# AndrewJarrett/raytracing-with-zig

Measured on NVIDIA B200. Metric: Msamples/s, higher is better.
Workload: dtype f32

## Files before the change

raytracing-with-zig_b200/csrc/rtz_api.cu:

```cuda
#include <cuda_runtime.h>
#include <dlfcn.h>
#include <nccl.h>

#include <algorithm>
#include <cerrno>
#include <cmath>
#include <cstdint>
#include <cstdio>
#include <cstdlib>
#include <cstring>
#include <condition_variable>
#include <functional>
#include <map>
#include <mutex>
#include <thread>
#include <memory>
#include <string>
#include <vector>

#include "../../include/rtz.h"
#include "rtz_kernels.cuh"
#include "rtz_bvh.cuh"
#include "rtz_scene.cuh"

// ... 193 lines not shown
    RTZ_CUDA(ctx->accum.reserve(3 * n_local_pixels));
    rtz::TraceParams P;
    P.cam = to_dev_camera(*cam, seed);
    P.sh = sg;
    P.geom = ctx->geom.p, P.pairs = ctx->pairs.p, P.aux = ctx->aux.p, P.albedo = ctx->albedo.p, P.wexp = ctx->wexp.p;
    P.orig = nullptr;
    P.n_spheres = ctx->n_spheres, P.n_pad = ctx->n_pad;
    pick_chunks(ctx, P, n_local_pixels);
    P.accum = ctx->accum.p;
    P.counter = ctx->counters.p;
    P.stats = ctx->counters.p + 1;
    {
        P.wave_shade_min = P.wave_regen_min = ctx->n_pad <= 32 ? 16u : ctx->n_pad <= 64 ? 12u : 8u;
        auto rcp = [](uint64_t d) -> unsigned long long {
            return d <= 1 ? 0ull : (unsigned long long)(((unsigned __int128)1 << 64) / d) + 1ull;
        };
        P.rcp_tile_pixels = rcp(sg.tile_pixels), P.rcp_tiles_x = rcp(sg.tiles_x), P.rcp_tile_w = rcp(sg.tile_w);
        P.rcp_chunks_per_pixel = rcp(P.chunks_per_pixel);
        if (const char* e = std::getenv("RTZ_WAVE_SHADE_MIN")) P.wave_shade_min = (uint32_t)std::min(32, std::max(1, std::atoi(e)));
        if (const char* e = std::getenv("RTZ_WAVE_REGEN_MIN")) P.wave_regen_min = (uint32_t)std::min(32, std::max(1, std::atoi(e)));
    }
    P.timeline = nullptr;
    if (const char* e = std::getenv("RTZ_TIMELINE")) {
        if (e[0] == '1') {
            RTZ_CUDA(ctx->timeline.reserve(4 * 65536));
            RTZ_CUDA(cudaMemsetAsync(ctx->timeline.p, 0, 4 * 65536 * sizeof(unsigned long long), ctx->stream));
            P.timeline = ctx->timeline.p;
        }
    }
    P.pool = nullptr, P.pool_count = reinterpret_cast<unsigned int*>(ctx->counters.p + 8);
    const char* de = std::getenv("RTZ_DRAIN");
    const bool drain = cam->mode == RTZ_MODE_PATH && ctx->variant != 4 && P.cam.bounce_max > 0 && !(de && de[0] == '0');
    if (drain) {
        RTZ_CUDA(ctx->pool.reserve(4ull * 64 * 32 * (size_t)ctx->sm_count * 2));
        P.pool = ctx->pool.p;
    }
    const bool use_const = ctx->n_pad <= rtz::kMaxConstSpheres && ctx->geo_const;
    const size_t smem = use_const ? 0 : (size_t)ctx->n_pad * 32;
    cudaFuncAttributes fa{};
    RTZ_CUDA(cudaFuncGetAttributes(&fa, rtz::trace_kernel_smem<512, 1>));
    const bool use_global = !use_const && smem + fa.sharedSizeBytes + 1024 > ctx->smem_optin;
    RTZ_CUDA(cudaEventRecord(ctx->ev[0], ctx->stream));
    RTZ_CUDA(cudaMemsetAsync(ctx->accum.p, 0, 3 * n_local_pixels * sizeof(unsigned long long), ctx->stream));
    RTZ_CUDA(cudaMemsetAsync(ctx->counters.p, 0, 16 * sizeof(unsigned long long), ctx->stream));
    RTZ_CUDA(cudaEventRecord(ctx->ev[1], ctx->stream));
    ctx->frame_launches = P.cam.bounce_max == 0 ? 1 : 2;
    int32_t rc = RTZ_OK;
    if (P.cam.bounce_max == 0) {
    } else if (cam->mode == RTZ_MODE_PATH_BVH) {
        rtz::BvhParams B{P, ctx->bvh_nodes.p, ctx->bvh_order.p, ctx->wexp.p};
        rc = launch_trace(ctx, rtz::trace_kernel_bvh<128, 6>, B, P.n_chunks, 128, 0);
    } else if (use_const) {
        static thread_local rtz::TraceParamsConst C;
        C.p = P;
        std::memcpy(C.pairs, ctx->h_pairs.data(), (size_t)ctx->n_pad * sizeof(float4));
        const bool wave_ok = P.n_chunks <= 0xFFFFFFFFull;
        if (ctx->variant == 4)
            rc = launch_trace(ctx, rtz::trace_kernel_const_parked<4, 128, 6>, C, P.n_chunks, 128, 0);
        else if (ctx->variant == 1)
            rc = launch_trace(ctx, rtz::trace_kernel_const<256, 3>, C, P.n_chunks, 256, 0);
        else if (ctx->variant == 2)
            rc = launch_trace(ctx, rtz::trace_kernel_const<128, 5>, C, P.n_chunks, 128, 0);
        else if (ctx->variant == 6)
            rc = launch_trace(ctx, rtz::trace_kernel_const<128, 7>, C, P.n_chunks, 128, 0);
        else if (ctx->variant == 7)
            rc = launch_trace(ctx, rtz::trace_kernel_const<128, 8>, C, P.n_chunks, 128, 0);
        else if (ctx->variant == 9 && wave_ok)
            rc = launch_trace(ctx, rtz::trace_kernel_wave<128, 10>, C, P.n_chunks, 128, 0);
        else if (ctx->variant == 10 && wave_ok)
            rc = launch_trace(ctx, rtz::trace_kernel_wave<128, 9>, C, P.n_chunks, 128, 0);
        else if (wave_ok && (ctx->variant == 8 || (ctx->variant == 0 && ctx->n_pad <= 32)))
            rc = launch_trace(ctx, rtz::trace_kernel_wave<128, 8>, C, P.n_chunks, 128, 0);
        else if (wave_ok && (ctx->variant == 12 || (ctx->variant == 0 && ctx->n_pad <= rtz::kMaxWaveSpheres)))
            rc = launch_trace(ctx, rtz::trace_kernel_wave_n<4, 128, 6>, C, P.n_chunks, 128, 0);
        else if (ctx->n_pad <= 64)
            rc = launch_trace(ctx, rtz::trace_kernel_const<128, 8>, C, P.n_chunks, 128, 0);
        else if (ctx->cull) {
            P.geom = ctx->rg_geom.p, P.aux = ctx->rg_aux.p, P.albedo = ctx->rg_albedo.p, P.wexp = ctx->rg_wexp.p;
            P.orig = ctx->rg_orig.p, P.pairs = nullptr;
            C.p = P;
            std::memcpy(C.pairs, ctx->h_rg_pairs.data(), (size_t)ctx->n_pad * sizeof(float4));
            std::memcpy(C.boxes, ctx->h_boxes.data(), ctx->h_boxes.size() * sizeof(float4));
            C.cull_r2 = ctx->cull_r2;
            rc = launch_trace(ctx, rtz::trace_kernel_const_cull<128, 6>, C, P.n_chunks, 128, 0);
        } else
            rc = launch_trace(ctx, rtz::trace_kernel_const<128, 6>, C, P.n_chunks, 128, 0);
    } else if (use_global) {
        rc = launch_trace(ctx, rtz::trace_kernel_global<128, 5>, P, P.n_chunks, 128, 0);
    } else {
        int occ[3] = {0, 0, 0};
        RTZ_CUDA(cudaFuncSetAttribute(rtz::trace_kernel_smem<128, 5>, cudaFuncAttributeMaxDynamicSharedMemorySize, (int)smem));
        RTZ_CUDA(cudaFuncSetAttribute(rtz::trace_kernel_smem<256, 2>, cudaFuncAttributeMaxDynamicSharedMemorySize, (int)smem));
        RTZ_CUDA(cudaFuncSetAttribute(rtz::trace_kernel_smem<512, 1>, cudaFuncAttributeMaxDynamicSharedMemorySize, (int)smem));
        RTZ_CUDA(cudaOccupancyMaxActiveBlocksPerMultiprocessor(&occ[0], rtz::trace_kernel_smem<128, 5>, 128, smem));
        RTZ_CUDA(cudaOccupancyMaxActiveBlocksPerMultiprocessor(&occ[1], rtz::trace_kernel_smem<256, 2>, 256, smem));
        RTZ_CUDA(cudaOccupancyMaxActiveBlocksPerMultiprocessor(&occ[2], rtz::trace_kernel_smem<512, 1>, 512, smem));
        const int warps[3] = {occ[0] * 4, occ[1] * 8, occ[2] * 16};
        int shape = 0;
        for (int k = 1; k < 3; ++k)
            if (warps[k] > warps[shape]) shape = k;
        if (ctx->variant >= 1 && ctx->variant <= 3) shape = ctx->variant - 1;
        switch (shape) {
            case 1: rc = launch_trace(ctx, rtz::trace_kernel_smem<256, 2>, P, P.n_chunks, 256, smem); break;
            case 2: rc = launch_trace(ctx, rtz::trace_kernel_smem<512, 1>, P, P.n_chunks, 512, smem); break;
            default: rc = launch_trace(ctx, rtz::trace_kernel_smem<128, 5>, P, P.n_chunks, 128, smem); break;
        }
    }
    if (rc != RTZ_OK) return rc;
    if (drain) {
        const unsigned blocks = (unsigned)ctx->sm_count * 8;
        if (ctx->n_spheres >= 64)
            rtz::drain_kernel<true><<<blocks, 128, 0, ctx->stream>>>(P);
        else
            rtz::drain_kernel<false><<<blocks, 128, 0, ctx->stream>>>(P);
        RTZ_CUDA(cudaGetLastError());
        ctx->frame_launches += 1;
    }
    RTZ_CUDA(cudaEventRecord(ctx->ev[2], ctx->stream));
    const uint64_t n3 = 3 * n_local_pixels;
    if (out.image)
        rtz::resolve_scatter_kernel<<<(unsigned)((n3 + 255) / 256), 256, 0, ctx->stream>>>(
            ctx->accum.p, sg, (uint32_t)cam->width, (uint32_t)cam->height, cam->pixel_samples_scale, out.image);
    else
        rtz::resolve_kernel<<<(unsigned)((n3 + 255) / 256), 256, 0, ctx->stream>>>(
            ctx->accum.p, n_local_pixels, cam->pixel_samples_scale, out.d_rgb, out.d_linear);
    RTZ_CUDA(cudaGetLastError());
    RTZ_CUDA(cudaEventRecord(ctx->ev[3], ctx->stream));
    RTZ_CUDA(cudaMemcpyAsync(ctx->h_counters, ctx->counters.p, 8 * sizeof(unsigned long long), cudaMemcpyDeviceToHost,
                             ctx->stream));
    return RTZ_OK;
}

int32_t collect_path(rtz_context* ctx, const rtz_camera* cam, const rtz::ShardGeom& sg, rtz_stats* st, uint64_t seed) {
    RTZ_CUDA(cudaStreamSynchronize(ctx->stream));
    if (const char* path = std::getenv("RTZ_TIMELINE_OUT")) {
        if (ctx->timeline.p && std::getenv("RTZ_TIMELINE") && std::getenv("RTZ_TIMELINE")[0] == '1') {
            std::vector<unsigned long long> h(4 * 65536);
            RTZ_CUDA(cudaMemcpy(h.data(), ctx->timeline.p, h.size() * sizeof(unsigned long long), cudaMemcpyDeviceToHost));
            if (FILE* f = std::fopen(path, "wb")) {
                std::fwrite(h.data(), sizeof(unsigned long long), h.size(), f);
                std::fclose(f);
            }
        }
    }
    if (st) {
        std::memset(st, 0, sizeof(*st));
        st->samples = ctx->h_counters[1], st->segments = ctx->h_counters[2];
        if (cam->bounce_max == 0) {
            uint64_t px = 0;
            for (uint32_t t = sg.rank; t < (uint64_t)sg.tiles_x * sg.tiles_y; t += sg.world) {
                const uint32_t ty = t / sg.tiles_x, tx = t - ty * sg.tiles_x;
                const uint64_t w = std::min<uint64_t>(sg.tile_w, cam->width - (uint64_t)tx * sg.tile_w);
                const uint64_t h = std::min<uint64_t>(sg.tile_h, cam->height - (uint64_t)ty * sg.tile_h);
                px += w * h;
            }
            st->samples = px * cam->samples_per_pixel;
        }
        st->depth_capped = ctx->h_counters[3], st->absorbed = ctx->h_counters[4];
        st->sphere_tests = cam->mode == RTZ_MODE_PATH_BVH ? ctx->h_counters[5] : st->segments * (uint64_t)ctx->n_spheres;
        st->nan_samples = ctx->h_counters[6];
        st->kernel_launches = ctx->frame_launches;
        st->gpus = 1;
        float ms = 0;
        cudaEventElapsedTime(&ms, ctx->ev[1], ctx->ev[2]), st->trace_ms = ms;
        cudaEventElapsedTime(&ms, ctx->ev[2], ctx->ev[3]), st->resolve_ms = ms;
        cudaEventElapsedTime(&ms, ctx->ev[0], ctx->ev[3]), st->total_ms = ms;
// ... 1096 lines not shown
```

raytracing-with-zig_b200/csrc/rtz_kernels.cuh:

```cuda
#pragma once
#include "rtz_device.cuh"

namespace rtz {

struct ShardGeom {
    uint32_t rank, world, tile_w, tile_h, tiles_x, tiles_y, n_local_tiles, tile_pixels;
};

struct TraceParams {
    DevCamera cam;
    ShardGeom sh;
    const float4* pairs;
    const float4* geom;
    const float4* aux;
    const float4* albedo;
    const float* wexp;
    const int* orig;
    int n_spheres;
    int n_pad;
    uint32_t chunk;
    uint32_t chunks_per_pixel;
    uint32_t n_local_pixels;
    uint64_t n_chunks;
    unsigned long long* accum;
    unsigned long long* counter;
    unsigned long long* stats;
    float4* pool;
    unsigned int* pool_count;
    unsigned long long* timeline;
    uint32_t wave_shade_min, wave_regen_min;
    unsigned long long rcp_tile_pixels, rcp_tiles_x, rcp_tile_w, rcp_chunks_per_pixel;
};

constexpr int kMaxConstSpheres = 512;
struct TraceParamsConst {
    TraceParams p;
    float4 pairs[kMaxConstSpheres];
    float4 boxes[2 * (kMaxConstSpheres / 32)];
    float cull_r2;
};

__device__ __forceinline__ bool local_to_global(const ShardGeom& s, uint32_t W, uint32_t H, uint32_t lp, uint32_t& x,
                                                uint32_t& y) {
    const uint32_t lt = lp / s.tile_pixels, within = lp - lt * s.tile_pixels;
    const uint32_t gt = lt * s.world + s.rank;
    const uint32_t ty = gt / s.tiles_x, tx = gt - ty * s.tiles_x;
    const uint32_t wy = within / s.tile_w, wx = within - wy * s.tile_w;
    x = tx * s.tile_w + wx, y = ty * s.tile_h + wy;
    return x < W && y < H && ty < s.tiles_y;
}

__device__ __forceinline__ uint32_t div_by(uint32_t n, unsigned long long rcp) {
    return rcp ? (uint32_t)__umul64hi((unsigned long long)n, rcp) : n;
}
__device__ __forceinline__ bool local_to_global_rcp(const ShardGeom& s, unsigned long long rcp_tile_pixels,
                                                    unsigned long long rcp_tiles_x, unsigned long long rcp_tile_w, uint32_t W,
                                                    uint32_t H, uint32_t lp, uint32_t& x, uint32_t& y) {
    const uint32_t lt = div_by(lp, rcp_tile_pixels), within = lp - lt * s.tile_pixels;
    const uint32_t gt = lt * s.world + s.rank;
    const uint32_t ty = div_by(gt, rcp_tiles_x), tx = gt - ty * s.tiles_x;
    const uint32_t wy = div_by(within, rcp_tile_w), wx = within - wy * s.tile_w;
    x = tx * s.tile_w + wx, y = ty * s.tile_h + wy;
    return x < W && y < H && ty < s.tiles_y;
}

__device__ __forceinline__ uint32_t smem_u32(const void* p) { return (uint32_t)__cvta_generic_to_shared(p); }
__device__ __forceinline__ void mbar_init(uint64_t* bar, uint32_t count) {
    asm volatile("mbarrier.init.shared::cta.b64 [%0], %1;" ::"r"(smem_u32(bar)), "r"(count));
}
__device__ __forceinline__ void mbar_expect_tx(uint64_t* bar, uint32_t bytes) {
    asm volatile("mbarrier.arrive.expect_tx.shared::cta.b64 _, [%0], %1;" ::"r"(smem_u32(bar)), "r"(bytes) : "memory");
}
__device__ __forceinline__ void bulk_g2s(void* dst, const void* src, uint32_t bytes, uint64_t* bar) {
    asm volatile("cp.async.bulk.shared::cluster.global.mbarrier::complete_tx::bytes [%0], [%1], %2, [%3];" ::"r"(
                     smem_u32(dst)),
                 "l"(src), "r"(bytes), "r"(smem_u32(bar))
                 : "memory");
}
__device__ __forceinline__ void mbar_wait(uint64_t* bar, uint32_t phase) {
    asm volatile(
        "{\n"
        ".reg .pred p;\n"
        "WAIT_%=:\n"
        "mbarrier.try_wait.parity.shared::cta.b64 p, [%0], %1;\n"
        "@p bra DONE_%=;\n"
        "bra WAIT_%=;\n"
        "DONE_%=:\n"
        "}\n" ::"r"(smem_u32(bar)),
        "r"(phase)
        : "memory");
}

struct Slot {
    Path path;
    RngKey key;
    uint32_t lp;
    bool alive;
};


__device__ __forceinline__ void resolve_candidates(const float4* __restrict__ gather, unsigned cand, int base, int cnt,
                                                   const Path& p, float tmin_d, float& closest, int& best,
                                                   const int* __restrict__ orig = nullptr) {
    while (cand) {
        const int bit = 31 - __clz(cand);
        cand &= ~(1u << bit);
        const int i = base + (cnt - 1 - bit);
        const float4 g = gather[i];
        candidate_root(g, g.w, i, p, tmin_d, closest, best, orig);
    }
}

__device__ __forceinline__ void test_pair(const float4 p0, const float4 p1, const Path& p, const RayK& k,
                                          unsigned& mask) {
    const float2 cx = make_float2(p0.x, p0.y), cy = make_float2(p0.z, p0.w);
    const float2 cz = make_float2(p1.x, p1.y), cw = make_float2(p1.z, p1.w);
    float2 h = __ffma2_rn(make_float2(p.dx, p.dx), cx, make_float2(k.k1, k.k1));
    h = __ffma2_rn(make_float2(p.dy, p.dy), cy, h);
    h = __ffma2_rn(make_float2(p.dz, p.dz), cz, h);
    float2 w = __ffma2_rn(make_float2(k.tx, k.tx), cx, make_float2(k.nk2, k.nk2));
    w = __ffma2_rn(make_float2(k.ty, k.ty), cy, w);
    w = __ffma2_rn(make_float2(k.tz, k.tz), cz, w);
    w = __fadd2_rn(w, cw);
    const float2 disc = __ffma2_rn(h, h, w);
    mask = __funnelshift_l(__float_as_uint(disc.x), mask, 1);
    mask = __funnelshift_l(__float_as_uint(disc.y), mask, 1);
}

__device__ __forceinline__ bool box_reach(const float4 b0, const float4 b1, const Path& p, float ix, float iy, float iz,
                                          float closest) {
    const float2 tx = __fmul2_rn(__fadd2_rn(make_float2(b0.x, b0.y), make_float2(-p.ox, -p.ox)), make_float2(ix, ix));
    const float2 ty = __fmul2_rn(__fadd2_rn(make_float2(b0.z, b0.w), make_float2(-p.oy, -p.oy)), make_float2(iy, iy));
    const float2 tz = __fmul2_rn(__fadd2_rn(make_float2(b1.x, b1.y), make_float2(-p.oz, -p.oz)), make_float2(iz, iz));
    const float tn = fmaxf(fmaxf(fminf(tx.x, tx.y), fminf(ty.x, ty.y)), fmaxf(fminf(tz.x, tz.y), 0.0f));
    const float tf = fminf(fminf(fmaxf(tx.x, tx.y), fmaxf(ty.x, ty.y)), fminf(fmaxf(tz.x, tz.y), closest));
    return tn <= tf;
}

template <bool kConstBank, bool kSkipSelf = false, bool kCull = false>
__device__ __forceinline__ void sweep2(const float4* __restrict__ pairs, const float4* __restrict__ gather, int n_pad,
                                       float tmin, float tmax, const Path& a, const Path& b, float& ta, int& ia,
                                       float& tb, int& ib, const float4* __restrict__ boxes = nullptr,
                                       float cull_r2 = 0.0f, const int* __restrict__ orig = nullptr) {
    RayK ka = ray_constants(a), kb = ray_constants(b);
    if (kConstBank && !kCull) asm volatile("" : "+f"(ka.tx), "+f"(ka.ty), "+f"(ka.tz), "+f"(kb.tx), "+f"(kb.ty), "+f"(kb.tz));
    float ca = tmax * a.len, cb = tmax * b.len;
    int ba = -1, bb = -1;
    float iax = 0.f, iay = 0.f, iaz = 0.f, ibx = 0.f, iby = 0.f, ibz = 0.f;
    if (kCull) {
        iax = 1.0f / a.dx, iay = 1.0f / a.dy, iaz = 1.0f / a.dz;
        ibx = 1.0f / b.dx, iby = 1.0f / b.dy, ibz = 1.0f / b.dz;
        if (!(-ka.nk2 <= cull_r2)) iax = iay = iaz = __int_as_float(0x7fffffff);
        if (!(-kb.nk2 <= cull_r2)) ibx = iby = ibz = __int_as_float(0x7fffffff);
    }
    for (int base = 0; base < n_pad; base += 32) {
        if (kCull && base > 0) {
            const float4 b0 = boxes[base >> 4], b1 = boxes[(base >> 4) + 1];
            const bool need = box_reach(b0, b1, a, iax, iay, iaz, ca) | box_reach(b0, b1, b, ibx, iby, ibz, cb);
            if (!__any_sync(0xFFFFFFFFu, need)) continue;
        }
        const int cnt = min(32, n_pad - base);
        unsigned ma = 0xFFFFFFFFu, mb = 0xFFFFFFFFu;
        const float4* g = pairs + base;
#pragma unroll 1
        for (int k = 0; k < cnt; k += 8) {
#pragma unroll
            for (int u = 0; u < 8; u += 2) {
                const float4 p0 = g[k + u], p1 = g[k + u + 1];
                test_pair(p0, p1, a, ka, ma);
                test_pair(p0, p1, b, kb, mb);
            }
        }
        unsigned canda = ~ma, candb = ~mb;
        if (kSkipSelf) {
            const unsigned ra = (unsigned)(a.self & ~kSelfLeaves) - (unsigned)base, rb = (unsigned)(b.self & ~kSelfLeaves) - (unsigned)base;
            if ((a.self >> 30) == 1 && ra < (unsigned)cnt) canda &= ~(1u << (cnt - 1 - (int)ra));
            if ((b.self >> 30) == 1 && rb < (unsigned)cnt) candb &= ~(1u << (cnt - 1 - (int)rb));
        }
        if (canda | candb) {
            float la = a.len, lb = b.len;
            if (!kConstBank) asm volatile("" : "+f"(la), "+f"(lb));
            resolve_candidates(gather, canda, base, cnt, a, tmin * la, ca, ba, orig);
            resolve_candidates(gather, candb, base, cnt, b, tmin * lb, cb, bb, orig);
        }
    }
    ta = ca, ia = ba, tb = cb, ib = bb;
}

__device__ __forceinline__ void finish_or_continue(const TraceParams& P, const float4* gather, const float4* s_aux,
                                                   const float4* s_alb, Slot& s, float t, int best,
                                                   unsigned long long& n_seg, uint32_t& n_samp, uint32_t& n_cap,
                                                   uint32_t& n_abs) {
    ++n_seg;
    float sr, sg, sb;
    int term;
    if (shade(P.cam, s.key, gather, s_aux, s_alb, s.path, t, best, sr, sg, sb, term)) {
        const unsigned long long fr = to_fixed(sr), fg = to_fixed(sg), fb = to_fixed(sb);
        unsigned long long* px = P.accum + 3ull * s.lp;
        if (fr) atomicAdd(px + 0, fr);
        if (fg) atomicAdd(px + 1, fg);
        if (fb) atomicAdd(px + 2, fb);
        if (sr != sr || sg != sg || sb != sb) atomicAdd(P.stats + 5, 1ULL);
        ++n_samp;
        n_cap += (term == 2), n_abs += (term == 1);
        s.alive = false;
    }
}

__device__ __forceinline__ void finish_or_continue(const TraceParams& P, const float4* gather, const float4* s_aux,
                                                   const float4* s_alb, Slot& s, float t, int best) {
    float sr, sg, sb;
    int term;
    if (shade(P.cam, s.key, gather, s_aux, s_alb, s.path, t, best, sr, sg, sb, term)) {
        const unsigned long long fr = to_fixed(sr), fg = to_fixed(sg), fb = to_fixed(sb);
        unsigned long long* px = P.accum + 3ull * s.lp;
        if (fr) atomicAdd(px + 0, fr);
        if (fg) atomicAdd(px + 1, fg);
        if (fb) atomicAdd(px + 2, fb);
        if (sr != sr || sg != sg || sb != sb) atomicAdd(P.stats + 5, 1ULL);
        if (term == 2) atomicAdd(P.stats + 2, 1ULL);
        if (term == 1) atomicAdd(P.stats + 3, 1ULL);
        s.alive = false;
    }
}

__device__ __forceinline__ unsigned long long globaltimer_ns() {
    unsigned long long t;
    asm volatile("mov.u64 %0, %globaltimer;" : "=l"(t));
    return t;
}

template <bool kUniform = false>
__device__ __forceinline__ void coop_hit(const float4* __restrict__ geom, const float* __restrict__ wexp,
                                         const int* __restrict__ orig, int n, float tmin, float tmax, const Path& mine,
                                         int src, unsigned lane, float& t_out, int& best_out) {
    Path q = mine;
    if (!kUniform) {
        q.ox = __shfl_sync(0xFFFFFFFFu, mine.ox, src), q.oy = __shfl_sync(0xFFFFFFFFu, mine.oy, src);
        q.oz = __shfl_sync(0xFFFFFFFFu, mine.oz, src), q.dx = __shfl_sync(0xFFFFFFFFu, mine.dx, src);
        q.dy = __shfl_sync(0xFFFFFFFFu, mine.dy, src), q.dz = __shfl_sync(0xFFFFFFFFu, mine.dz, src);
        q.len = __shfl_sync(0xFFFFFFFFu, mine.len, src), q.self = __shfl_sync(0xFFFFFFFFu, mine.self, src);
    }
    const float tmin_d = tmin * q.len;
    float closest = tmax * q.len;
    int best = -1;
    const RayK k = ray_constants(q);
    for (int base = (int)lane; base < n; base += 256) {
        unsigned cand = 0u;
#pragma unroll
        for (int j = 0; j < 8; ++j) {
            const int i = base + 32 * j;
            if (i < n) {
                const float4 g = __ldg(geom + i);
                const float d = expanded_disc(g.x, g.y, g.z, __ldg(wexp + i), q, k);
                cand |= (__float_as_uint(d) >> 31 ^ 1u) << j;
            }
        }
        while (cand) {
            const int j = __ffs(cand) - 1;
            cand &= cand - 1u;
            const int i = base + 32 * j;
            const float4 g = __ldg(geom + i);
            candidate_root(g, g.w, i, q, tmin_d, closest, best, orig);
        }
    }
#pragma unroll
    for (int o = 16; o > 0; o >>= 1) {
        const float t2 = __shfl_xor_sync(0xFFFFFFFFu, closest, o);
        const int b2 = __shfl_xor_sync(0xFFFFFFFFu, best, o);
        const bool tie_won = t2 == closest && b2 >= 0 && (best < 0 || (orig ? __ldg(orig + b2) < __ldg(orig + best) : b2 < best));
        if (t2 < closest || tie_won) closest = t2, best = b2;
    }
    if (kUniform || (int)lane == src) t_out = closest, best_out = best;
}

__device__ __forceinline__ void park_path(float4* __restrict__ e, const Slot& s) {
    const Path& p = s.path;
    e[0] = make_float4(p.ox, p.oy, p.oz, p.len);
    e[1] = make_float4(p.dx, p.dy, p.dz, __int_as_float(p.self));
    e[2] = make_float4(p.tr, p.tg, p.tb, __uint_as_float(p.bounce));
    e[3] = make_float4(__uint_as_float(s.key.pixel), __uint_as_float(s.key.sample), __uint_as_float(s.lp), 0.f);
}
__device__ __forceinline__ void unpark_path(const float4* __restrict__ e, uint32_t k0, uint32_t k1, Slot& s) {
    const float4 a = e[0], b = e[1], c = e[2], d = e[3];
    Path& p = s.path;
    p.ox = a.x, p.oy = a.y, p.oz = a.z, p.len = a.w;
    p.dx = b.x, p.dy = b.y, p.dz = b.z, p.self = __float_as_int(b.w);
    p.tr = c.x, p.tg = c.y, p.tb = c.z, p.bounce = __float_as_uint(c.w);
    s.key = RngKey{k0, k1, __float_as_uint(d.x), __float_as_uint(d.y)};
    s.lp = __float_as_uint(d.z);
    s.alive = true;
}

__device__ __forceinline__ void take_camera_ray(const float* stage, uint32_t j, Path& p) {
    p.ox = stage[0 * 64 + j], p.oy = stage[1 * 64 + j], p.oz = stage[2 * 64 + j];
    p.dx = stage[3 * 64 + j], p.dy = stage[4 * 64 + j], p.dz = stage[5 * 64 + j];
    p.len = stage[6 * 64 + j];
    p.tr = p.tg = p.tb = 1.0f;
    p.self = -1;
    p.bounce = 0;
}
constexpr int kStageFloats = 7 * 64;

template <bool kConstBank, int kBlock, bool kCull = false>
__device__ __forceinline__ void trace_body(const TraceParams& P, const float4* __restrict__ pairs,
                                           const float4* __restrict__ gather, float* __restrict__ stage_mem,
                                           const float4* __restrict__ boxes = nullptr, float cull_r2 = 0.0f) {
    float* const stage = stage_mem + (threadIdx.x >> 5) * kStageFloats;
    unsigned long long* const tl =
        P.timeline ? P.timeline + 4ull * ((unsigned long long)blockIdx.x * (kBlock / 32) + (threadIdx.x >> 5)) : nullptr;
    if (tl && (threadIdx.x & 31u) == 0u) tl[0] = globaltimer_ns();
    const float4* s_aux = P.aux;
    const float4* s_alb = P.albedo;
    const unsigned lane = threadIdx.x & 31u;
    const unsigned lt_mask = (1u << lane) - 1u;
    const DevCamera& cam = P.cam;

    Slot A, B;
    A.alive = B.alive = false;
    A.lp = B.lp = 0;
    A.key = B.key = RngKey{cam.key0, cam.key1, 0u, 0u};
    A.path.ox = A.path.oy = A.path.oz = 0.f, A.path.dx = A.path.dy = 0.f, A.path.dz = 1.f;
    A.path.tr = A.path.tg = A.path.tb = 0.f, A.path.len = 1.f, A.path.self = -1, A.path.bounce = 0;
    B.path = A.path;

    uint32_t ch_lp = 0, ch_x = 0, ch_y = 0, ch_next = 0, ch_end = 0;
    bool exhausted = false;

    unsigned long long n_seg = 0;
    uint32_t n_samp = 0;
    unsigned prev_a = 0u, prev_b = 0u;

    for (;;) {
        unsigned need_a = __ballot_sync(0xFFFFFFFFu, !A.alive);
        unsigned need_b = __ballot_sync(0xFFFFFFFFu, !B.alive);
        n_samp += __popc(prev_a & need_a) + __popc(prev_b & need_b);
        if (need_a | need_b) {
            while ((need_a | need_b) && !exhausted) {
                if (ch_next >= ch_end) {
                    unsigned long long cid = 0;
                    if (lane == 0) cid = atomicAdd(P.counter, 1ULL);
                    cid = __shfl_sync(0xFFFFFFFFu, cid, 0);
                    if (__any_sync(0xFFFFFFFFu, cid >= P.n_chunks)) {
                        exhausted = true;
                        if (tl && lane == 0u) tl[1] = globaltimer_ns();
                        break;
                    }
                    const uint32_t lp = (uint32_t)(cid / P.chunks_per_pixel);
                    const uint32_t part = (uint32_t)(cid - (unsigned long long)lp * P.chunks_per_pixel);
                    uint32_t x, y;
                    const bool inside = local_to_global(P.sh, cam.width, cam.height, lp, x, y);
                    if (__any_sync(0xFFFFFFFFu, !inside)) continue;
                    ch_lp = lp, ch_x = x, ch_y = y;
                    ch_next = part * P.chunk;
                    ch_end = min(ch_next + P.chunk, cam.spp);
                }
                const uint32_t avail = ch_end - ch_next;
                const uint32_t na = __popc(need_a);
                const uint32_t rank_a = __popc(need_a & lt_mask);
                const uint32_t rank_b = na + __popc(need_b & lt_mask);
                const uint32_t n_gen = min(na + (uint32_t)__popc(need_b), avail);
                const uint32_t pix = ch_y * cam.width + ch_x;
                for (uint32_t j0 = 0; j0 < n_gen; j0 += 32u) {
                    const uint32_t j = j0 + lane;
                    if (j < n_gen) {
                        const RngKey key{cam.key0, cam.key1, pix, ch_next + j};
                        Path t;
                        camera_ray(cam, key, ch_x, ch_y, t);
                        stage[0 * 64 + j] = t.ox, stage[1 * 64 + j] = t.oy, stage[2 * 64 + j] = t.oz;
                        stage[3 * 64 + j] = t.dx, stage[4 * 64 + j] = t.dy, stage[5 * 64 + j] = t.dz;
                        stage[6 * 64 + j] = t.len;
                    }
                }
                __syncwarp();
                if (((need_a >> lane) & 1u) && rank_a < n_gen) {
                    A.lp = ch_lp;
                    A.key.pixel = pix, A.key.sample = ch_next + rank_a;
                    take_camera_ray(stage, rank_a, A.path);
                    A.alive = true;
                }
                if (((need_b >> lane) & 1u) && rank_b < n_gen) {
                    B.lp = ch_lp;
                    B.key.pixel = pix, B.key.sample = ch_next + rank_b;
                    take_camera_ray(stage, rank_b, B.path);
                    B.alive = true;
                }
                __syncwarp();
                ch_next += n_gen;
                need_a = __ballot_sync(0xFFFFFFFFu, !A.alive);
                need_b = __ballot_sync(0xFFFFFFFFu, !B.alive);
            }
        }
        if (exhausted && P.pool) {
            const unsigned pa = __ballot_sync(0xFFFFFFFFu, A.alive), pb = __ballot_sync(0xFFFFFFFFu, B.alive);
            unsigned base = 0u;
            if (lane == 0u) base = atomicAdd(P.pool_count, (unsigned)(__popc(pa) + __popc(pb)));
            base = __shfl_sync(0xFFFFFFFFu, base, 0);
            if (A.alive) park_path(P.pool + 4ull * (base + __popc(pa & lt_mask)), A);
            if (B.alive) park_path(P.pool + 4ull * (base + __popc(pa) + __popc(pb & lt_mask)), B);
            break;
        }
        const unsigned live_a = __ballot_sync(0xFFFFFFFFu, A.alive), live_b = __ballot_sync(0xFFFFFFFFu, B.alive);
        if ((live_a | live_b) == 0u) break;
        n_seg += (unsigned)(__popc(live_a) + __popc(live_b));
        prev_a = live_a, prev_b = live_b;
        float ta = 0.f, tb = 0.f;
        int ia = -1, ib = -1;
        sweep2<kConstBank, false, kCull>(pairs, gather, P.n_pad, cam.tmin, cam.tmax, A.path, B.path, ta, ia, tb, ib,
                                         boxes, cull_r2, kCull ? P.orig : nullptr);
        if (A.alive) finish_or_continue(P, gather, s_aux, s_alb, A, ta, ia);
        if (B.alive) finish_or_continue(P, gather, s_aux, s_alb, B, tb, ib);
        __syncwarp();
    }
    if (tl && lane == 0u) {
        unsigned smid;
        asm volatile("mov.u32 %0, %smid;" : "=r"(smid));
        tl[2] = globaltimer_ns(), tl[3] = smid;
    }
    if (lane == 0u) {
        atomicAdd(P.stats + 0, (unsigned long long)n_samp);
        atomicAdd(P.stats + 1, n_seg);
    }
}

enum ParkField { kOx, kOy, kOz, kDx, kDy, kDz, kTr, kTg, kTb, kLen, kSelf, kBounce, kPixel, kSample, kLp, kParkFields };

template <int R, int kBlock>
struct Park {
    float* base;
    __device__ __forceinline__ float& f(int field, int slot) const {
        return base[(field * R + slot) * kBlock + threadIdx.x];
    }
    __device__ __forceinline__ uint32_t& u(int field, int slot) const {
        return reinterpret_cast<uint32_t*>(base)[(field * R + slot) * kBlock + threadIdx.x];
    }
    __device__ __forceinline__ float fv(int field, int slot) const {
        return *reinterpret_cast<volatile float*>(&base[(field * R + slot) * kBlock + threadIdx.x]);
    }
    __device__ __forceinline__ void store_ray(int s, const Path& p) const {
        f(kOx, s) = p.ox, f(kOy, s) = p.oy, f(kOz, s) = p.oz;
        f(kDx, s) = p.dx, f(kDy, s) = p.dy, f(kDz, s) = p.dz;
        f(kTr, s) = p.tr, f(kTg, s) = p.tg, f(kTb, s) = p.tb;
        f(kLen, s) = p.len, u(kSelf, s) = (uint32_t)p.self, u(kBounce, s) = p.bounce;
    }
    __device__ __forceinline__ void load_ray(int s, Path& p) const {
        p.ox = f(kOx, s), p.oy = f(kOy, s), p.oz = f(kOz, s);
        p.dx = f(kDx, s), p.dy = f(kDy, s), p.dz = f(kDz, s);
        p.tr = f(kTr, s), p.tg = f(kTg, s), p.tb = f(kTb, s);
        p.len = f(kLen, s), p.self = (int)u(kSelf, s), p.bounce = u(kBounce, s);
    }
};

struct Hot {
    float dx, dy, dz, k1, tx, ty, tz, nk2;
};

__device__ __forceinline__ void test_pair_hot(const float4 p0, const float4 p1, const Hot& q, unsigned& mask) {
    const float2 cx = make_float2(p0.x, p0.y), cy = make_float2(p0.z, p0.w);
    const float2 cz = make_float2(p1.x, p1.y), cw = make_float2(p1.z, p1.w);
    float2 h = __ffma2_rn(make_float2(q.dx, q.dx), cx, make_float2(q.k1, q.k1));
    h = __ffma2_rn(make_float2(q.dy, q.dy), cy, h);
    h = __ffma2_rn(make_float2(q.dz, q.dz), cz, h);
    float2 w = __ffma2_rn(make_float2(q.tx, q.tx), cx, make_float2(q.nk2, q.nk2));
    w = __ffma2_rn(make_float2(q.ty, q.ty), cy, w);
    w = __ffma2_rn(make_float2(q.tz, q.tz), cz, w);
    w = __fadd2_rn(w, cw);
    const float2 disc = __ffma2_rn(h, h, w);
    mask = __funnelshift_l(__float_as_uint(disc.x), mask, 1);
    mask = __funnelshift_l(__float_as_uint(disc.y), mask, 1);
}

template <int R, int kBlock>
__device__ __forceinline__ void trace_body_parked(const TraceParams& P, const float4* __restrict__ pairs,
                                                  const float4* __restrict__ gather, float* park_mem,
                                                  uint8_t* todo_mem) {
    const Park<R, kBlock> park{park_mem};
    uint8_t* todo = todo_mem + (threadIdx.x >> 5) * (32 * R);
    const float4* s_aux = P.aux;
    const float4* s_alb = P.albedo;
    const unsigned lane = threadIdx.x & 31u;
    const unsigned lt_mask = (1u << lane) - 1u;
    const DevCamera& cam = P.cam;
    constexpr unsigned kFull = (1u << R) - 1u;

    unsigned alive = 0;
    {
        Path idle;
        idle.ox = idle.oy = idle.oz = 0.f, idle.dx = idle.dy = 0.f, idle.dz = 1.f;
        idle.tr = idle.tg = idle.tb = 0.f, idle.len = 1.f, idle.self = -1, idle.bounce = 0;
#pragma unroll
        for (int s = 0; s < R; ++s) park.store_ray(s, idle);
    }

    uint32_t ch_lp = 0, ch_x = 0, ch_y = 0, ch_next = 0, ch_end = 0;
    bool exhausted = false;
    unsigned long long n_seg = 0;
    uint32_t n_samp = 0, n_cap = 0, n_abs = 0;
// ... 80 lines not shown
                    for (int s = 0; s < R; ++s) test_pair_hot(p0, p1, hot[s], m[s]);
                }
            }
            unsigned any = 0;
#pragma unroll
            for (int s = 0; s < R; ++s) any |= ~m[s];
            if (any) {
#pragma unroll
                for (int s = 0; s < R; ++s) {
                    if (~m[s]) {
                        Path p;
                        p.ox = park.fv(kOx, s), p.oy = park.fv(kOy, s), p.oz = park.fv(kOz, s);
                        p.dx = hot[s].dx, p.dy = hot[s].dy, p.dz = hot[s].dz;
                        p.self = __float_as_int(park.fv(kSelf, s));
                        const float tmin_d = cam.tmin * park.fv(kLen, s);
                        resolve_candidates(gather, ~m[s], base, cnt, p, tmin_d, closest[s], best[s]);
                    }
                }
            }
        }

#pragma unroll 1
        for (int s = 0; s < R; ++s) {
            float t = closest[0];
            int b = best[0];
#pragma unroll
            for (int q = 1; q < R; ++q)
                if (s == q) t = closest[q], b = best[q];
            if ((alive >> s) & 1u) {
                ++n_seg;
                Path p;
                park.load_ray(s, p);
                const RngKey key{cam.key0, cam.key1, park.u(kPixel, s), park.u(kSample, s)};
                float sr, sg, sb;
                int term;
                if (shade(cam, key, gather, s_aux, s_alb, p, t, b, sr, sg, sb, term)) {
                    const unsigned long long fr = to_fixed(sr), fg = to_fixed(sg), fb = to_fixed(sb);
                    unsigned long long* px = P.accum + 3ull * park.u(kLp, s);
                    if (fr) atomicAdd(px + 0, fr);
                    if (fg) atomicAdd(px + 1, fg);
                    if (fb) atomicAdd(px + 2, fb);
                    if (sr != sr || sg != sg || sb != sb) atomicAdd(P.stats + 5, 1ULL);
                    ++n_samp;
                    n_cap += (term == 2), n_abs += (term == 1);
                    alive &= ~(1u << s);
                } else {
                    park.store_ray(s, p);
                }
            }
            __syncwarp();
        }
    }
    unsigned long long v0 = n_samp, v1 = n_seg, v2 = n_cap, v3 = n_abs;
#pragma unroll
    for (int o = 16; o > 0; o >>= 1) {
        v0 += __shfl_xor_sync(0xFFFFFFFFu, v0, o);
        v1 += __shfl_xor_sync(0xFFFFFFFFu, v1, o);
        v2 += __shfl_xor_sync(0xFFFFFFFFu, v2, o);
        v3 += __shfl_xor_sync(0xFFFFFFFFu, v3, o);
    }
    if (lane == 0) {
        atomicAdd(P.stats + 0, v0);
        atomicAdd(P.stats + 1, v1);
        atomicAdd(P.stats + 2, v2);
        atomicAdd(P.stats + 3, v3);
    }
}

template <int R, int kBlock, int kMinBlocks>
__global__ void __launch_bounds__(kBlock, kMinBlocks) trace_kernel_const_parked(const __grid_constant__ TraceParamsConst C) {
    __shared__ float park_mem[kParkFields * R * kBlock];
    __shared__ uint8_t todo_mem[kBlock * R];
    trace_body_parked<R, kBlock>(C.p, C.pairs, C.p.geom, park_mem, todo_mem);
}

template <int kBlock, int kMinBlocks>
__global__ void __launch_bounds__(kBlock, kMinBlocks) trace_kernel_const(const __grid_constant__ TraceParamsConst C) {
    __shared__ float stage[(kBlock / 32) * kStageFloats];
    trace_body<true, kBlock>(C.p, C.pairs, C.p.geom, stage);
}

template <int kBlock, int kMinBlocks>
__global__ void __launch_bounds__(kBlock, kMinBlocks) trace_kernel_const_cull(const __grid_constant__ TraceParamsConst C) {
    __shared__ float stage[(kBlock / 32) * kStageFloats];
    trace_body<true, kBlock, true>(C.p, C.pairs, C.p.geom, stage, C.boxes, C.cull_r2);
}

template <int kBlock, int kMinBlocks>
__global__ void __launch_bounds__(kBlock, kMinBlocks) trace_kernel_smem(const __grid_constant__ TraceParams P) {
    extern __shared__ __align__(128) unsigned char smem_raw[];
    float4* s_pairs = reinterpret_cast<float4*>(smem_raw);
    float4* s_geom = s_pairs + P.n_pad;
    __shared__ __align__(8) uint64_t s_bar;
    __shared__ float stage[(kBlock / 32) * kStageFloats];
    if (threadIdx.x == 0) {
        mbar_init(&s_bar, 1);
        asm volatile("fence.mbarrier_init.release.cluster;" ::: "memory");
    }
    __syncthreads();
    if (threadIdx.x == 0) {
        const uint32_t bytes = (uint32_t)P.n_pad * 16u;
        mbar_expect_tx(&s_bar, 2u * bytes);
        bulk_g2s(s_pairs, P.pairs, bytes, &s_bar);
        bulk_g2s(s_geom, P.geom, bytes, &s_bar);
    }
    mbar_wait(&s_bar, 0);
    trace_body<false, kBlock>(P, s_pairs, s_geom, stage);
}

template <int kBlock, int kMinBlocks>
__global__ void __launch_bounds__(kBlock, kMinBlocks) trace_kernel_global(const __grid_constant__ TraceParams P) {
    __shared__ float stage[(kBlock / 32) * kStageFloats];
    trace_body<false, kBlock>(P, P.pairs, P.geom, stage);
}

enum WaveField { wOx, wOy, wOz, wDx, wDy, wDz, wLen, wSelf, wTr, wTg, wTb, wBounce, wSample, wPixel, wLp, wT, wBest, kWaveFields };
constexpr int kMaxWaveSpheres = 256;
constexpr int kWaveWords = kWaveFields * 64 + 32;

__device__ __forceinline__ void wave_add_sky(const TraceParams& P, const float* w, const uint32_t* wu, uint32_t s) {
    const float al = 0.5f * (w[wDy * 64 + s] + 1.0f);
    const float wh = 1.0f - al;
    const float sr = w[wTr * 64 + s] * fmaf(al, 0.5f, wh);
    const float sg = w[wTg * 64 + s] * fmaf(al, 0.7f, wh);
    const float sb = w[wTb * 64 + s] * fmaf(al, 1.0f, wh);
    const unsigned long long fr = to_fixed(sr), fg = to_fixed(sg), fb = to_fixed(sb);
    unsigned long long* px = P.accum + 3ull * wu[wLp * 64 + s];
    if (fr) atomicAdd(px + 0, fr);
    if (fg) atomicAdd(px + 1, fg);
    if (fb) atomicAdd(px + 2, fb);
    if (sr != sr || sg != sg || sb != sb) atomicAdd(P.stats + 5, 1ULL);
}
constexpr uint32_t kWaveSky = 0xFFFFFFFFu;
constexpr uint32_t kWaveEnded = 0xFFFFFFFEu;

template <int kBlock>
__device__ __forceinline__ void trace_body_wave(const TraceParams& P, const float4* __restrict__ pairs,
                                                const float4* __restrict__ gather, float* __restrict__ wave_mem) {
    float* const w = wave_mem + (threadIdx.x >> 5) * kWaveWords;
    uint32_t* const wu = reinterpret_cast<uint32_t*>(w);
    uint8_t* const hit_list = reinterpret_cast<uint8_t*>(w + kWaveFields * 64);
    uint8_t* const free_list = hit_list + 64;
    const unsigned lane = threadIdx.x & 31u;
    const unsigned lt_mask = (1u << lane) - 1u;
    const DevCamera& cam = P.cam;
    const uint32_t sa = lane, sb = lane + 32u;

    w[wOx * 64 + sa] = w[wOy * 64 + sa] = w[wOz * 64 + sa] = 0.f, w[wDx * 64 + sa] = w[wDy * 64 + sa] = 0.f;
    w[wDz * 64 + sa] = 1.f, w[wLen * 64 + sa] = 1.f, wu[wSelf * 64 + sa] = 0xFFFFFFFFu;
    w[wOx * 64 + sb] = w[wOy * 64 + sb] = w[wOz * 64 + sb] = 0.f, w[wDx * 64 + sb] = w[wDy * 64 + sb] = 0.f;
    w[wDz * 64 + sb] = 1.f, w[wLen * 64 + sb] = 1.f, wu[wSelf * 64 + sb] = 0xFFFFFFFFu;
    wu[wBest * 64 + sa] = kWaveEnded, wu[wBest * 64 + sb] = kWaveEnded;
    __syncwarp();

    bool alive_a = false, alive_b = false;
    uint32_t ch_lp = 0, ch_x = 0, ch_y = 0, ch_next = 0, ch_end = 0;
    bool exhausted = false;
    unsigned long long n_seg = 0;
    uint32_t n_samp = 0, flip = 0;

    for (;;) {
        if (!exhausted) {
            const unsigned fa = __ballot_sync(0xFFFFFFFFu, !alive_a), fb = __ballot_sync(0xFFFFFFFFu, !alive_b);
            const uint32_t nfa = __popc(fa), n_free = nfa + __popc(fb);
            const uint32_t rem = n_free & 31u;
            const uint32_t n_fill = (n_free - rem) + (rem >= P.wave_regen_min ? rem : 0u);
            if (n_fill) {
                const uint32_t rank_a = __popc(fa & lt_mask), rank_b = nfa + __popc(fb & lt_mask);
// ... 755 lines not shown
```

Baseline: 4719.

## Transpose sparse culled sphere-group tests across lanes when few rays need them

```diff
diff --git a/raytracing-with-zig_b200/csrc/rtz_api.cu b/raytracing-with-zig_b200/csrc/rtz_api.cu
--- a/raytracing-with-zig_b200/csrc/rtz_api.cu
+++ b/raytracing-with-zig_b200/csrc/rtz_api.cu
@@ -299,6 +299,8 @@
             std::memcpy(C.pairs, ctx->h_rg_pairs.data(), (size_t)ctx->n_pad * sizeof(float4));
             std::memcpy(C.boxes, ctx->h_boxes.data(), ctx->h_boxes.size() * sizeof(float4));
             C.cull_r2 = ctx->cull_r2;
+            C.split_max = rtz::kSplitMax;
+            if (const char* e = std::getenv("RTZ_SPLIT")) C.split_max = std::atoi(e);
             rc = launch_trace(ctx, rtz::trace_kernel_const_cull<128, 6>, C, P.n_chunks, 128, 0);
         } else
             rc = launch_trace(ctx, rtz::trace_kernel_const<128, 6>, C, P.n_chunks, 128, 0);
diff --git a/raytracing-with-zig_b200/csrc/rtz_kernels.cuh b/raytracing-with-zig_b200/csrc/rtz_kernels.cuh
--- a/raytracing-with-zig_b200/csrc/rtz_kernels.cuh
+++ b/raytracing-with-zig_b200/csrc/rtz_kernels.cuh
@@ -38,7 +38,9 @@
     float4 pairs[kMaxConstSpheres];
     float4 boxes[2 * (kMaxConstSpheres / 32)];
     float cull_r2;
+    int split_max;
 };
+constexpr int kSplitMax = 16;
 
 __device__ __forceinline__ bool local_to_global(const ShardGeom& s, uint32_t W, uint32_t H, uint32_t lp, uint32_t& x,
                                                 uint32_t& y) {
@@ -137,11 +139,37 @@
     return tn <= tf;
 }
 
+__device__ __forceinline__ float4 lds_opaque(const float4* p) {
+    float4 v;
+    asm volatile("ld.shared.v4.f32 {%0, %1, %2, %3}, [%4];" : "=f"(v.x), "=f"(v.y), "=f"(v.z), "=f"(v.w) : "r"(smem_u32(p))
+                 : "memory");
+    return v;
+}
+
+__device__ __forceinline__ unsigned split_candidates(const float4* __restrict__ stage, unsigned need, const float4 g,
+                                                     float w, unsigned lane) {
+    unsigned cand = 0u;
+    while (need) {
+        const unsigned src = __ffs(need) - 1;
+        need &= need - 1u;
+        const float4 s0 = stage[2 * src], s1 = stage[2 * src + 1];
+        Path q;
+        q.dx = s1.y, q.dy = s1.z, q.dz = s1.w;
+        const RayK k{s0.x, s0.y, s0.z, s0.w, s1.x};
+        const float d = expanded_disc(g.x, g.y, g.z, w, q, k);
+        const unsigned pass = __ballot_sync(0xFFFFFFFFu, !(__float_as_uint(d) >> 31));
+        if (lane == src) cand = pass;
+    }
+    return cand;
+}
+
 template <bool kConstBank, bool kSkipSelf = false, bool kCull = false>
 __device__ __forceinline__ void sweep2(const float4* __restrict__ pairs, const float4* __restrict__ gather, int n_pad,
                                        float tmin, float tmax, const Path& a, const Path& b, float& ta, int& ia,
                                        float& tb, int& ib, const float4* __restrict__ boxes = nullptr,
-                                       float cull_r2 = 0.0f, const int* __restrict__ orig = nullptr) {
+                                       float cull_r2 = 0.0f, const int* __restrict__ orig = nullptr,
+                                       const float* __restrict__ wexp = nullptr, int split_max = 0,
+                                       float4* __restrict__ stage = nullptr) {
     RayK ka = ray_constants(a), kb = ray_constants(b);
     if (kConstBank && !kCull) asm volatile("" : "+f"(ka.tx), "+f"(ka.ty), "+f"(ka.tz), "+f"(kb.tx), "+f"(kb.ty), "+f"(kb.tz));
     float ca = tmax * a.len, cb = tmax * b.len;
@@ -153,25 +181,54 @@
         if (!(-ka.nk2 <= cull_r2)) iax = iay = iaz = __int_as_float(0x7fffffff);
         if (!(-kb.nk2 <= cull_r2)) ibx = iby = ibz = __int_as_float(0x7fffffff);
     }
+    if (kCull) {
+        const unsigned lane = threadIdx.x & 31u;
+        stage[2 * lane] = make_float4(ka.k1, ka.nk2, ka.tx, ka.ty);
+        stage[2 * lane + 1] = make_float4(ka.tz, a.dx, a.dy, a.dz);
+        stage[2 * lane + 64] = make_float4(kb.k1, kb.nk2, kb.tx, kb.ty);
+        stage[2 * lane + 65] = make_float4(kb.tz, b.dx, b.dy, b.dz);
+        stage[2 * lane + 128] = make_float4(iax, iay, iaz, 0.f);
+        stage[2 * lane + 129] = make_float4(ibx, iby, ibz, 0.f);
+        __syncwarp();
+    }
     for (int base = 0; base < n_pad; base += 32) {
+        unsigned canda, candb;
+        unsigned need_a = 0u, need_b = 0u;
         if (kCull && base > 0) {
             const float4 b0 = boxes[base >> 4], b1 = boxes[(base >> 4) + 1];
-            const bool need = box_reach(b0, b1, a, iax, iay, iaz, ca) | box_reach(b0, b1, b, ibx, iby, ibz, cb);
-            if (!__any_sync(0xFFFFFFFFu, need)) continue;
+            need_a = __ballot_sync(0xFFFFFFFFu, box_reach(b0, b1, a, iax, iay, iaz, ca));
+            need_b = __ballot_sync(0xFFFFFFFFu, box_reach(b0, b1, b, ibx, iby, ibz, cb));
+            if ((need_a | need_b) == 0u) continue;
         }
         const int cnt = min(32, n_pad - base);
-        unsigned ma = 0xFFFFFFFFu, mb = 0xFFFFFFFFu;
-        const float4* g = pairs + base;
+        if (kCull && base > 0 && __popc(need_a) + __popc(need_b) <= split_max) {
+            const unsigned lane = threadIdx.x & 31u;
+            const int i = min(base + (int)lane, n_pad - 1);
+            const float4 g = gather[i];
+            const float w = __ldg(wexp + i);
+            canda = split_candidates(stage, need_a, g, w, lane);
+            candb = split_candidates(stage + 64, need_b, g, w, lane);
+            canda = __brev(canda) >> (32 - cnt);
+            candb = __brev(candb) >> (32 - cnt);
+            const float4 a0 = lds_opaque(stage + 2 * lane), a1 = lds_opaque(stage + 2 * lane + 1);
+            const float4 b0 = lds_opaque(stage + 2 * lane + 64), b1 = lds_opaque(stage + 2 * lane + 65);
+            const float4 ra = lds_opaque(stage + 2 * lane + 128), rb = lds_opaque(stage + 2 * lane + 129);
+            ka = RayK{a0.x, a0.y, a0.z, a0.w, a1.x}, kb = RayK{b0.x, b0.y, b0.z, b0.w, b1.x};
+            iax = ra.x, iay = ra.y, iaz = ra.z, ibx = rb.x, iby = rb.y, ibz = rb.z;
+        } else {
+            unsigned ma = 0xFFFFFFFFu, mb = 0xFFFFFFFFu;
+            const float4* g = pairs + base;
 #pragma unroll 1
-        for (int k = 0; k < cnt; k += 8) {
-#pragma unroll
-            for (int u = 0; u < 8; u += 2) {
-                const float4 p0 = g[k + u], p1 = g[k + u + 1];
-                test_pair(p0, p1, a, ka, ma);
-                test_pair(p0, p1, b, kb, mb);
-            }
-        }
-        unsigned canda = ~ma, candb = ~mb;
+            for (int k = 0; k < cnt; k += 8) {
+#pragma unroll
+                for (int u = 0; u < 8; u += 2) {
+                    const float4 p0 = g[k + u], p1 = g[k + u + 1];
+                    test_pair(p0, p1, a, ka, ma);
+                    test_pair(p0, p1, b, kb, mb);
+                }
+            }
+            canda = ~ma, candb = ~mb;
+        }
         if (kSkipSelf) {
             const unsigned ra = (unsigned)(a.self & ~kSelfLeaves) - (unsigned)base, rb = (unsigned)(b.self & ~kSelfLeaves) - (unsigned)base;
             if ((a.self >> 30) == 1 && ra < (unsigned)cnt) canda &= ~(1u << (cnt - 1 - (int)ra));
@@ -301,15 +358,22 @@
     p.bounce = 0;
 }
 constexpr int kStageFloats = 7 * 64;
+constexpr int kCullStageFloats = 12 * 64;
+
+template <int kBlock>
+__device__ __forceinline__ unsigned long long* timeline_row(const TraceParams& P) {
+    unsigned cta;
+    asm volatile("mov.u32 %0, %%ctaid.x;" : "=r"(cta));
+    return P.timeline + 4ull * ((unsigned long long)cta * (kBlock / 32) + (threadIdx.x >> 5));
+}
 
 template <bool kConstBank, int kBlock, bool kCull = false>
 __device__ __forceinline__ void trace_body(const TraceParams& P, const float4* __restrict__ pairs,
                                            const float4* __restrict__ gather, float* __restrict__ stage_mem,
-                                           const float4* __restrict__ boxes = nullptr, float cull_r2 = 0.0f) {
-    float* const stage = stage_mem + (threadIdx.x >> 5) * kStageFloats;
-    unsigned long long* const tl =
-        P.timeline ? P.timeline + 4ull * ((unsigned long long)blockIdx.x * (kBlock / 32) + (threadIdx.x >> 5)) : nullptr;
-    if (tl && (threadIdx.x & 31u) == 0u) tl[0] = globaltimer_ns();
+                                           const float4* __restrict__ boxes = nullptr, float cull_r2 = 0.0f,
+                                           int split_max = 0) {
+    float* const stage = stage_mem + (threadIdx.x >> 5) * (kCull ? kCullStageFloats : kStageFloats);
+    if (P.timeline && (threadIdx.x & 31u) == 0u) timeline_row<kBlock>(P)[0] = globaltimer_ns();
     const float4* s_aux = P.aux;
     const float4* s_alb = P.albedo;
     const unsigned lane = threadIdx.x & 31u;
@@ -343,7 +407,7 @@
                     cid = __shfl_sync(0xFFFFFFFFu, cid, 0);
                     if (__any_sync(0xFFFFFFFFu, cid >= P.n_chunks)) {
                         exhausted = true;
-                        if (tl && lane == 0u) tl[1] = globaltimer_ns();
+                        if (P.timeline && lane == 0u) timeline_row<kBlock>(P)[1] = globaltimer_ns();
                         break;
                     }
                     const uint32_t lp = (uint32_t)(cid / P.chunks_per_pixel);
@@ -407,12 +471,14 @@
         float ta = 0.f, tb = 0.f;
         int ia = -1, ib = -1;
         sweep2<kConstBank, false, kCull>(pairs, gather, P.n_pad, cam.tmin, cam.tmax, A.path, B.path, ta, ia, tb, ib,
-                                         boxes, cull_r2, kCull ? P.orig : nullptr);
+                                         boxes, cull_r2, kCull ? P.orig : nullptr, P.wexp, split_max,
+                                         reinterpret_cast<float4*>(stage));
         if (A.alive) finish_or_continue(P, gather, s_aux, s_alb, A, ta, ia);
         if (B.alive) finish_or_continue(P, gather, s_aux, s_alb, B, tb, ib);
         __syncwarp();
     }
-    if (tl && lane == 0u) {
+    if (P.timeline && lane == 0u) {
+        unsigned long long* const tl = timeline_row<kBlock>(P);
         unsigned smid;
         asm volatile("mov.u32 %0, %smid;" : "=r"(smid));
         tl[2] = globaltimer_ns(), tl[3] = smid;
@@ -659,8 +725,8 @@
 
 template <int kBlock, int kMinBlocks>
 __global__ void __launch_bounds__(kBlock, kMinBlocks) trace_kernel_const_cull(const __grid_constant__ TraceParamsConst C) {
-    __shared__ float stage[(kBlock / 32) * kStageFloats];
-    trace_body<true, kBlock, true>(C.p, C.pairs, C.p.geom, stage, C.boxes, C.cull_r2);
+    __shared__ __align__(16) float stage[(kBlock / 32) * kCullStageFloats];
+    trace_body<true, kBlock, true>(C.p, C.pairs, C.p.geom, stage, C.boxes, C.cull_r2, C.split_max);
 }
 
 template <int kBlock, int kMinBlocks>
```

Result: faster. 5570, median of 6 (+18.0%).
